# LauraFJulia/TFT_vs_Fund

Measured on AMD Instinct MI355X. Metric: triplet-hypotheses/sec (linearTFT+R,t) at N=200 corresp., higher is better.
Workload: dtype f64; 1 GPU; configs[1]: batch of 10000 synthetic triplets x 200 correspondences, sigma=1px, linearTFT + R_t_from_TFT (LinearTFTPoseEstimation without Reconst), one batch per GPU; batch_per_gpu=10000, correspondences=200, streams=2 (consecutive batches alternate between streams and may overlap), gather=none (1 GPU), failed_triplets=0, warmup_steps_run=2560

## Files before the change

tft_vs_fund_amd/csrc/gh_rows_kernel.h:

```cpp
#pragma once
#include "tft_rows_kernel.h"
#include "tft_rows_exact_kernel.h"
#include "gh_wg_kernel.h"

namespace tff {

template <bool PRE>
__global__ void __launch_bounds__(64, 2) k_gh_linear_rows(const GhWgArgs a) {
    TFF_DYNAMIC_LDS(double, smem);
    const int lane = lane_id();
    const int p = lane & 15, row = lane >> 4;
    RowLds* w = reinterpret_cast<RowLds*>(smem) + row;
    for (long blk = blockIdx.x; blk * ROW_TRIPLETS < a.B; blk += gridDim.x) {
        const int N = opaque_int(a.N);
        const long b_raw = blk * ROW_TRIPLETS + row;
        const bool valid = b_raw < a.B;
        const long b = valid ? b_raw : a.B - 1;
        RowSrc src;
        src.idx = nullptr; src.pts = a.corresp + b * 6 * (long)N; src.ns = 0; src.sampled = false;
        wave_sync();
        int status = ST_OK;
        if (N < 7) {
            status = ST_TOO_FEW;
        } else {
            if constexpr (PRE) {
                rows_load_pre(a.pre, b, w->mom, w->nrm);
            } else {
                double cen[6], nr[9];
                rows_centroids(src, N, cen);
                rows_distances_moments(src, N, cen, w->nrm, nr, w->mom);
            }
            wave_sync();
            const bool ok = rows_linear_tft_middle(w, nullptr, true);
            if (!ok) status = ST_RETRY;
            if (valid && ok) {
                double* r = a.rec + b * GH_REC_DOUBLES;
                r[p] = w->t[p];
                if (p < 11) r[16 + p] = w->t[16 + p];
                r[27 + p] = w->pa[p];
                if (p < 2) r[27 + 16 + p] = w->pa[16 + p];
                if (p < 6) r[45 + p] = w->epi[p];
                if (p < 9) r[51 + p] = w->nrm[p];
            }
        }
        if (p == 0 && valid) { a.status[b] = status; if (a.iter) a.iter[b] = 0; }
    }
}

__global__ void __launch_bounds__(64, 2) k_gh_finish_rows(const GhWgArgs a) {
    TFF_DYNAMIC_LDS(double, smem);
    const int lane = lane_id();
    const int p = lane & 15, row = lane >> 4;
    RowLds* w = reinterpret_cast<RowLds*>(smem) + row;
    RowRt* rt = reinterpret_cast<RowRt*>(w->ov);
    LinearTftArgs la{};
    la.corresp = a.corresp; la.calm = a.calm; la.calm_stride = a.calm_stride; la.B = a.B; la.N = a.N; la.flags = a.flags;
    la.Rt2 = a.Rt2; la.Rt3 = a.Rt3; la.T = a.T; la.reconst = a.reconst; la.iter = nullptr; la.status = a.status; la.dbg = nullptr;
    for (long blk = blockIdx.x; blk * ROW_TRIPLETS < a.B; blk += gridDim.x) {
        const int N = opaque_int(a.N);
        RowJob j;
        const long b_raw = blk * ROW_TRIPLETS + row;
        j.valid = b_raw < a.B;
        j.b = j.valid ? b_raw : a.B - 1;
        j.bad_index = false; j.dbg = nullptr;
        j.src.idx = nullptr; j.src.pts = a.corresp + j.b * 6 * (long)N; j.src.ns = 0; j.src.sampled = false;
        wave_sync();
        const int s0 = a.status[j.b];
        const bool dead = s0 > 0;
        if (dead) rows_store_nan(la, j, N);
        w->calm[p] = a.calm[j.b * a.calm_stride + p];
        if (p < 11) w->calm[16 + p] = a.calm[j.b * a.calm_stride + 16 + p];
        w->t[p] = dead ? ((p == 0) ? 1.0 : 0.0) : a.topt[j.b * 27 + p];
        if (p < 11) w->t[16 + p] = dead ? 0.0 : a.topt[j.b * 27 + 16 + p];
        if (p < 9) w->nrm[p] = dead ? ((p % 3 == 0) ? 1.0 : 0.0) : a.rec[j.b * GH_REC_DOUBLES + 51 + p];
        wave_sync();
        j.valid = j.valid && !dead;
        rows_transform_tft_inverse(w->t, rt->T1, rt->mats, [w](int v) { return normal_matrix(w->nrm, v); });
        bool ok = rows_rt_prepare<false>(w, rt, nullptr);
        int status = rows_pose_tail<false, false>(la, w, rt, j, N, ok);
        if (wave_any(status == ST_RETRY)) {
            RowJob jx = j;
            jx.valid = j.valid && status == ST_RETRY;
            wave_sync();
            rows_transform_tft_inverse(w->t, rt->T1, rt->mats, [w](int v) { return normal_matrix(w->nrm, v); });
            ok = rows_rt_prepare<true>(w, rt, nullptr);
            const int sx = rows_pose_tail<false, true>(la, w, rt, jx, N, ok);
            status = (status == ST_RETRY) ? sx : status;
        }
        if (s0 < 0) status = -s0;
        if (p == 0 && j.valid) a.status[j.b] = status;
    }
}

}
```

tft_vs_fund_amd/csrc/tft_rows_kernel.h:

```cpp
#pragma once
#include "tft_kernel.h"
#include "tft_moments_kernel.h"
#include <rows_target.h>
#include <regs_target.h>

namespace tff {

constexpr int ROW_TRIPLETS = 4;
constexpr int ROWL = 16;

struct RowRt {
    double T1[28];
    double T2[28];
    double nullv[18];
    double mats[28];
    double Ein[18];
    double cand[2][21];
    alignas(16) double P[4][12];
    alignas(16) double candRt[4][12];
    alignas(16) double Rt[2][12];
    alignas(16) double Pfin[3][12];
};
constexpr int ROW_OV_DOUBLES = 380;
static_assert(sizeof(RowRt) <= ROW_OV_DOUBLES * sizeof(double), "overlay");
struct alignas(16) RowLds {
    alignas(16) double mom[96];
    double nrm[9];
    double calm[27];
    double t[27];
    double epi[6];
    double Q[18];
    double tp[15];
    double pa[18];
    alignas(16) double ov[ROW_OV_DOUBLES];
};
static_assert(sizeof(RowLds) == (96 + 9 + 27 + 27 + 6 + 18 + 15 + 18 + ROW_OV_DOUBLES) * sizeof(double), "alignment adds no padding");
static_assert(sizeof(RowRt) == 318 * sizeof(double) && alignof(RowRt) == 16, "alignment adds no padding");
constexpr int ROW_LDS_DOUBLES = (int)(sizeof(RowLds) / sizeof(double));
static_assert(ROW_LDS_DOUBLES % 2 == 0, "16-byte row stride");
inline size_t rows_lds_bytes() { return (size_t)ROW_TRIPLETS * sizeof(RowLds); }
inline unsigned rows_grid(long B) { const long g = (B + ROW_TRIPLETS - 1) / ROW_TRIPLETS; return (unsigned)(g > 0 ? g : 1); }

__device__ __forceinline__ int rows_p() { return lane_id() & 15; }

struct RowSrc { const double* pts; const int* idx; int ns; bool sampled; };
__device__ __forceinline__ Pt6 rows_load(const RowSrc& s, const int i) {
    if (s.sampled) {
        int k = s.idx[i];
        k = (k >= 0 && k < s.ns) ? k : 0;
        return load_pt(s.pts, k);
    }
    return load_pt(s.pts, i);
}

__device__ __forceinline__ void rows_stamp(double* dbg, const int slot) {
    if (dbg) {
        const long long t = shader_clock();
        if (rows_p() == 0) dbg[80 + slot] = (double)t;
    }
}


__device__ __forceinline__ void rows_centroids(const RowSrc& s, const int N, double (&c)[6]) {
    const int p = rows_p();
    double sm[6] = {0, 0, 0, 0, 0, 0};
    int i0 = 0;
#pragma unroll 1
    for (; i0 + 4 * ROWL <= N; i0 += 4 * ROWL) {
        Pt6 q[4];
#pragma unroll
        for (int u = 0; u < 4; ++u) q[u] = rows_load(s, i0 + ROWL * u + p);
#pragma unroll
        for (int u = 0; u < 4; ++u)
#pragma unroll
            for (int k = 0; k < 6; ++k) sm[k] += q[u].v[k];
    }
    if (i0 < N) {
        Pt6 q[4];
#pragma unroll
        for (int u = 0; u < 4; ++u) { const int i = i0 + ROWL * u + p; q[u] = rows_load(s, (i < N) ? i : 0); }
#pragma unroll
        for (int u = 0; u < 4; ++u) {
            if (i0 + ROWL * u + p < N) {
#pragma unroll
                for (int k = 0; k < 6; ++k) sm[k] += q[u].v[k];
            }
        }
    }
#pragma unroll
    for (int k = 0; k < 6; ++k) c[k] = row_sum16(sm[k]) / (double)N;
}

__device__ __forceinline__ void rows_distances_moments(const RowSrc& s, const int N, const double (&c)[6], double* nrm, double (&nr)[9], double* mom) {
    const int p = rows_p();
    const int slot = p >> 1;
    const bool odd = (p & 1) != 0;
    double acc[48];
#pragma unroll
    for (int k = 0; k < 48; ++k) acc[k] = zero_f64();
    double dA = 0.0, dB = 0.0;
    auto body = [&](const Pt6& q, double& r2_out) {
        const double x1 = q.v[0] - c[0], y1 = q.v[1] - c[1];
        const double x2 = q.v[2] - c[2], y2 = q.v[3] - c[3];
        const double x3 = q.v[4] - c[4], y3 = q.v[5] - c[5];
        const double r1 = x1 * x1 + y1 * y1, r2 = x2 * x2 + y2 * y2, r3 = x3 * x3 + y3 * y3;
        dA += sqrt_nonneg_uniform(odd ? r3 : r1);
        r2_out = r2;
        const double q2[4] = {1.0, x2, y2, r2};
        const double q3[4] = {1.0, x3, y3, r3};
        const double pa = odd ? y1 * y1 : x1 * x1, pb = odd ? y1 : x1 * y1, pc = odd ? 1.0 : x1;
#pragma unroll
        for (int b = 0; b < 4; ++b)
#pragma unroll
            for (int cc = 0; cc < 4; ++cc) {
                const double wv = q3[b] * q2[cc];
                acc[4 * b + cc] += pa * wv;
                acc[16 + 4 * b + cc] += pb * wv;
                acc[32 + 4 * b + cc] += pc * wv;
            }
    };
    constexpr int STEP = ROWL / 2;
    Pt6 pe = rows_load(s, (slot < N) ? slot : 0);
    Pt6 po = rows_load(s, (slot + STEP < N) ? slot + STEP : 0);
#pragma unroll 1
    for (int i = slot; i < N; i += 2 * STEP) {
        const Pt6 q = pe;
        if (i + 2 * STEP < N) pe = rows_load(s, i + 2 * STEP);
        double r2a, r2b = 0.0;
        body(q, r2a);
        if (i + STEP < N) {
            const Pt6 r = po;
            if (i + 3 * STEP < N) po = rows_load(s, i + 3 * STEP);
            body(r, r2b);
        }
        dB += sqrt_nonneg_uniform(odd ? r2b : r2a);
    }
    const double d1 = row_sum16(odd ? 0.0 : dA), d3 = row_sum16(odd ? dA : 0.0), d2 = row_sum16(dB);
    const double r2c = sqrt(2.0);
    const double dd[3] = {d1, d2, d3};
#pragma unroll
    for (int v = 0; v < 3; ++v) {
        const double norm0 = dd[v] / (double)N;
        nr[3 * v + 0] = r2c / norm0;
        nr[3 * v + 1] = -r2c * c[2 * v] / norm0;
        nr[3 * v + 2] = -r2c * c[2 * v + 1] / norm0;
    }
    if (p == 0) {
#pragma unroll
        for (int k = 0; k < 9; ++k) nrm[k] = nr[k];
    }
    const bool up8 = (p & 8) != 0, up4 = (p & 4) != 0, up2 = (p & 2) != 0;
#pragma unroll
    for (int i = 0; i < 24; ++i) acc[i] = halve_sum<8>(acc[i], acc[i + 24], up8);
#pragma unroll
    for (int i = 0; i < 12; ++i) acc[i] = halve_sum<4>(acc[i], acc[i + 12], up4);
#pragma unroll
    for (int i = 0; i < 6; ++i) acc[i] = halve_sum<2>(acc[i], acc[i + 6], up2);
    const int base = 6 * ((p >> 1) & 1) + 12 * ((p >> 2) & 1) + 24 * ((p >> 3) & 1);
    const double s1 = nr[0], s2 = nr[3], s3 = nr[6];
#pragma unroll
    for (int i = 0; i < 6; ++i) {
        const int e = 48 * (p & 1) + base + i;
        const int h = e >> 4, i3 = (e >> 2) & 3, i2 = e & 3;
        const double f1 = (h == 5) ? 1.0 : ((h == 2 || h == 4) ? s1 : s1 * s1);
        const double f3 = (i3 == 0) ? 1.0 : ((i3 == 3) ? s3 * s3 : s3);
        const double f2 = (i2 == 0) ? 1.0 : ((i2 == 3) ? s2 * s2 : s2);
        mom[e] = acc[i] * (f1 * f3 * f2);
    }
}

template <int n>
__device__ __forceinline__ void rows_min_eigvec(double (&g0)[RowEigDims<n>::N0], double (&g1)[RowEigDims<n>::N1], const double d0, const double d1,
                                                double* Lp, const int maxit, int* iters, double* resid2, const bool has_start,
                                                const double start0, const double start1, double* gram_risk, double& x0, double& x1,
                                                const double gram_risk_limit2 = 1e14) {
    constexpr int N0 = RowEigDims<n>::N0;
    constexpr bool HI = RowEigDims<n>::HI;
    constexpr int Z = n * (n - 1) / 2;
    const int p = rows_p();
    const bool valid0 = p < n, valid1 = HI && 16 + p < n;
    const double tr = row_sum16((valid0 ? d0 : 0.0) + (valid1 ? d1 : 0.0));
    const double delta = 1e-14 * tr;
    const double pfloor = 1e-3 * delta + 1e-300;
    double myinv0 = 0.0, myinv1 = 0.0;
    RowChol<n, 0>::run(g0, g1, myinv0, myinv1, delta, pfloor, p);
#pragma unroll
    for (int c = 0; c < N0; ++c) g0[c] = (c < p && valid0) ? g0[c] * myinv0 : 0.0;
    if constexpr (HI) {
#pragma unroll
        for (int c = 0; c < n; ++c) g1[c] = ((c < 16 || c < 16 + p) && valid1) ? g1[c] * myinv1 : 0.0;
    }
    wave_sync();
    {
        const int t0 = (p * (p - 1)) / 2, t1 = ((16 + p) * (15 + p)) / 2;
#pragma unroll
        for (int c = 0; c < N0; ++c) Lp[(c < p && valid0) ? t0 + c : Z] = g0[c];
        if constexpr (HI) {
#pragma unroll
            for (int c = 0; c < n - 1; ++c) Lp[((c < 16 || c < 16 + p) && valid1) ? t1 + c : Z] = g1[c];
        }
    }
    wave_sync();
    x0 = valid0 ? rsqrt((double)n) : 0.0;
    x1 = valid1 ? rsqrt((double)n) : 0.0;
    if (has_start) {
        const double s0 = valid0 ? start0 : 0.0, s1 = valid1 ? start1 : 0.0;
        const double nn0 = row_sum16(s0 * s0 + s1 * s1);
        if (nn0 > 1e-300 && nn0 < 1e300) { const double r0 = rsqrt(nn0); x0 = s0 * r0; x1 = s1 * r0; }
    }
    double c0[n], c1[n];
#pragma unroll
    for (int j = 0; j < n; ++j) {
        c0[j] = Lp[(valid0 && p < j) ? (j * (j - 1)) / 2 + p : Z];
        c1[j] = (HI && j > 16) ? Lp[(valid1 && 16 + p < j) ? (j * (j - 1)) / 2 + 16 + p : Z] : 0.0;
    }
    double rprev2 = 1.0, res = 1.0, rk_r2 = 0.0, rk_rp = 1.0, rk_nn = 0.0;
    int it = 0;
    bool done = false;
#pragma unroll 1
    while (true) {
        double y0 = x0 * myinv0, y1 = x1 * myinv1;
        if constexpr (HI) {
            const double* rows = Lp + opaque_int(0);
            const int t0 = (p * (p - 1)) / 2;
#pragma unroll
            for (int c = 0; c < N0; ++c) g0[c] = rows[(c < p) ? t0 + c : Z];
        }
        RowForward<n, 0>::run(y0, y1, g0, g1);
        RowBackward<n, n - 1>::run(y0, y1, c0, c1);
        y0 *= myinv0; y1 *= myinv1;
        const double nn = row_sum16(y0 * y0 + y1 * y1);
        const double dot = row_sum16(y0 * x0 + y1 * x1);
        const double rn = rsqrt(nn);
        const double sc = (dot < 0.0) ? -rn : rn;
        const double yn0 = y0 * sc, yn1 = y1 * sc;
        const double dd0 = yn0 - x0, dd1 = yn1 - x1;
        const double r2 = row_sum16(dd0 * dd0 + dd1 * dd1);
        if (!done) {
            x0 = yn0; x1 = yn1;
            ++it;
            if (r2 <= 1e-26) { res = 0.0; done = true; }
            else if (it >= 2 && r2 < 0.25 * rprev2 && r2 * r2 < 1e-26 * rprev2) { res = 0.0; done = true; }
            else if (!(r2 == r2) || it >= maxit) { res = (r2 == r2) ? r2 : 1.0; done = true; }
            if (it >= 2 && r2 > 1e-30) { rk_r2 = r2; rk_rp = rprev2; rk_nn = nn; }
            rprev2 = r2;
        }
        if (!wave_any(!done)) break;
    }
    *iters = it;
    *resid2 = res;
    if (gram_risk) {
        const double num = 4.0 * rk_nn * rk_r2 * rk_rp;
        const double d = rk_rp - rk_r2;
        const double den = (rk_r2 < rk_rp) ? d * d : 0.0;
        *gram_risk = (tr * tr * num < gram_risk_limit2 * den) ? 0.0 : 1.0;
    }
}

template <class MatFn>
__device__ __forceinline__ void rows_transform_tft_inverse(const double* to, double* tn, double* mats, MatFn matrix_of) {
    const int p = rows_p();
    if (p < 3) {
        Mat3 M = matrix_of(p);
        if (p > 0) M = mat3_inv(M);
#pragma unroll
        for (int r = 0; r < 3; ++r)
#pragma unroll
            for (int c = 0; c < 3; ++c) mats[9 * p + 3 * r + c] = M.m[r][c];
    }
    wave_sync();
    double val[2];
#pragma unroll
    for (int h = 0; h < 2; ++h) {
        const int e = 16 * h + p;
        const bool have = e < 27;
        const int ee = have ? e : 0;
        const int i = ee / 9, k = (ee % 9) / 3, j = ee % 3;
        const double m0 = mats[i], m1 = mats[3 + i], m2 = mats[6 + i];
        double v = 0.0;
#pragma unroll
        for (int c = 0; c < 3; ++c)
#pragma unroll
            for (int d = 0; d < 3; ++d) {
                const double mix = m0 * to[c + 3 * d] + m1 * to[c + 3 * d + 9] + m2 * to[c + 3 * d + 18];
                v += mats[9 + 3 * j + c] * mix * mats[18 + 3 * k + d];
            }
        val[h] = have ? v : 0.0;
    }
    const double nn = row_sum16(val[0] * val[0] + val[1] * val[1]);
    const double rs = rsqrt(nn);
    wave_sync();
    tn[p] = val[0] * rs;
    if (p < 11) tn[16 + p] = val[1] * rs;
    wave_sync();
}

__device__ __forceinline__ bool rows_linear_tft_middle(RowLds* w, double* dbg, const bool want_P = false) {
    const int p = opaque_lane_int(rows_p());
    bool ok = true;
    int it1 = 0, it2 = 0;
    {
        const bool hi = p < 11;
        double ga[27], gb[27], g0[16], da, db, r2, risk, x0, x1;
        gram_row27(w->mom, p, ga, da);
        gram_row27(w->mom, hi ? 16 + p : 0, gb, db);
#pragma unroll
        for (int c = 0; c < 16; ++c) g0[c] = ga[c];
        rows_stamp(dbg, 3);
        rows_min_eigvec<27>(g0, gb, da, hi ? db : 0.0, w->ov, EIG_MAXIT, &it1, &r2, false, 0.0, 0.0, &risk, x0, x1);
        ok = ok && eig_converged(r2) && risk == 0.0;
        wave_sync();
        w->t[p] = x0;
        if (hi) w->t[16 + p] = x1;
        wave_sync();
    }
    if (dbg) { dbg[p] = w->t[p]; if (p < 11) dbg[16 + p] = w->t[16 + p]; }
    rows_stamp(dbg, 4);
    const bool eok = epipoles_from_tensor<16, false>(w->t, w->ov, w->epi, false);
    ok = !row_any(!eok) && ok;
    rows_stamp(dbg, 5);
    if (dbg && p < 6) dbg[27 + p] = w->epi[p];
    if (p < 2) frame_of(w->epi + 3 * p, w->Q + 9 * p);
    wave_sync();
    double* Gp = w->ov;
    constexpr GpIndexTable gp_index = make_gp_index_table();
    const unsigned long long gw0 = gp_index.w[rows_p()][0], gw1 = gp_index.w[rows_p()][1];
    int trip = 0;
#pragma unroll 1
    for (int e = p; e < 120; e += ROWL, ++trip) {
        const unsigned gw = (unsigned)(((trip < 4) ? gw0 : gw1) >> (16 * (trip & 3)));
        double a2[3], a3[3], b2[3], b3[3], c2[4], c3[4];
        up_factors_jk(w->Q, (int)(gw & 3u), (int)((gw >> 2) & 3u), a2, a3);
        up_factors_jk(w->Q, (int)((gw >> 4) & 3u), (int)((gw >> 6) & 3u), b2, b3);
        cvec(a2, b2, c2);
        cvec(a3, b3, c3);
        Gp[e] = bilinear44(w->mom + 16 * (int)((gw >> 8) & 7u), c3, c2);
    }
    wave_sync();
    rows_stamp(dbg, 6);
    {
        double g[15], none[1] = {0.0}, diag = 0.0, x0, x1, r2, risk;
        const bool have = p < 15;
        const int r = have ? p : 0;
#pragma unroll
        for (int c = 0; c < 15; ++c) g[c] = (c <= r && have) ? Gp[tri_index(r, c)] : 0.0;
        diag = Gp[tri_index(r, r)];
        double tp0 = 0.0;
        if (have) {
            const int i = r / 5, m = r % 5, jj = (m < 3) ? 0 : m - 2, kk = (m < 3) ? m : 0;
#pragma unroll
            for (int k = 0; k < 3; ++k)
#pragma unroll
                for (int j = 0; j < 3; ++j) tp0 += w->Q[3 * j + jj] * w->Q[9 + 3 * k + kk] * w->t[j + 3 * k + 9 * i];
        }
        wave_sync();
        rows_min_eigvec<15>(g, none, diag, 0.0, w->ov, EIG_MAXIT, &it2, &r2, true, tp0, 0.0, &risk, x0, x1);
        ok = ok && eig_converged(r2) && risk == 0.0;
        if (have) w->tp[p] = x0;
        wave_sync();
    }
    rows_stamp(dbg, 7);
    {
        double tv[2];
#pragma unroll
        for (int h = 0; h < 2; ++h) {
            const int e = (16 * h + p < 27) ? 16 * h + p : 0;
            const int i = e / 9, k = (e % 9) / 3, j = e % 3;
            double acc = 0.0;
#pragma unroll
            for (int m = 0; m < 5; ++m) {
                const int jj = (m < 3) ? 0 : m - 2, kk = (m < 3) ? m : 0;
                acc += w->Q[3 * j + jj] * w->Q[9 + 3 * k + kk] * w->tp[5 * i + m];
            }
            tv[h] = acc;
        }
        wave_sync();
        w->t[p] = tv[0];
        if (p < 11) w->t[16 + p] = tv[1];
        wave_sync();
    }
    if (dbg) {
        dbg[33 + p] = w->t[p];
        if (p < 11) dbg[33 + 16 + p] = w->t[16 + p];
        if (p == 0) { dbg[69] = (double)it1; dbg[70] = (double)it2; }
    }
    if (want_P) {
        if (p < 3) {
            const int i = p;
            const double* e21 = w->epi; const double* e31 = w->epi + 3;
            double ai[3], bi[3];
            for (int j = 0; j < 3; ++j) ai[j] = w->t[j + 9 * i] * e31[0] + w->t[j + 3 + 9 * i] * e31[1] + w->t[j + 6 + 9 * i] * e31[2];
            const double ae = ai[0] * e21[0] + ai[1] * e21[1] + ai[2] * e21[2];
            for (int k = 0; k < 3; ++k) {
                const double tte = w->t[3 * k + 9 * i] * e21[0] + w->t[1 + 3 * k + 9 * i] * e21[1] + w->t[2 + 3 * k + 9 * i] * e21[2];
                bi[k] = e31[k] * ae - tte;
            }
            const double be = bi[0] * e31[0] + bi[1] * e31[1] + bi[2] * e31[2];
            const double n21 = e21[0] * e21[0] + e21[1] * e21[1] + e21[2] * e21[2];
            const double n31 = e31[0] * e31[0] + e31[1] * e31[1] + e31[2] * e31[2];
            const double c = -(ae + be) / (n21 + n31);
            for (int j = 0; j < 3; ++j) { w->pa[3 * i + j] = ai[j] + c * e21[j]; w->pa[9 + 3 * i + j] = bi[j] + c * e31[j]; }
        }
        wave_sync();
    }
    return ok;
}

__device__ __forceinline__ void rows_recover_prepare(RowLds* w, RowRt* rt);
template <bool EXACT = false>
__device__ __forceinline__ bool rows_rt_prepare(RowLds* w, RowRt* rt, double* dbg) {
    const int p = rows_p();
    rows_transform_tft_inverse(rt->T1, rt->T2, rt->mats, [w](int v) { return load_K(w->calm, v); });
    const bool eok = epipoles_from_tensor<16, EXACT>(rt->T2, rt->nullv, w->epi, true);
    const bool ok = !row_any(!eok);
    if (p < 2) {
        const double* e21 = w->epi; const double* e31 = w->epi + 3;
        Mat3 M;
#pragma unroll
        for (int i = 0; i < 3; ++i)
#pragma unroll
            for (int r = 0; r < 3; ++r) {
                double acc = 0.0;
#pragma unroll
                for (int q = 0; q < 3; ++q) acc += (p == 0) ? rt->T2[r + 3 * q + 9 * i] * e31[q] : rt->T2[q + 3 * r + 9 * i] * e21[q];
                M.m[r][i] = acc;
            }
        const double* e = (p == 0) ? e21 : e31;
        const double sg = (p == 0) ? 1.0 : -1.0;
#pragma unroll
        for (int c = 0; c < 3; ++c) {
            rt->Ein[9 * p + 0 + c] = sg * (-e[2] * M.m[1][c] + e[1] * M.m[2][c]);
            rt->Ein[9 * p + 3 + c] = sg * (e[2] * M.m[0][c] - e[0] * M.m[2][c]);
            rt->Ein[9 * p + 6 + c] = sg * (-e[1] * M.m[0][c] + e[0] * M.m[1][c]);
        }
    }
    wave_sync();
    rows_stamp(dbg, 9);
    rows_recover_prepare(w, rt);
    return ok;
}

__device__ __forceinline__ void rows_recover_prepare(RowLds* w, RowRt* rt) {
    const int p = rows_p();
    if (p < 2) {
        Mat3 E, U, V;
#pragma unroll
        for (int r = 0; r < 3; ++r)
#pragma unroll
            for (int c = 0; c < 3; ++c) E.m[r][c] = rt->Ein[9 * p + 3 * r + c];
        double sv[3];
        svd3(E, U, V, sv);
        Mat3 UW, UWt, Vt = mat3_T(V);
#pragma unroll
        for (int r = 0; r < 3; ++r) {
            UW.m[r][0] = U.m[r][1];  UW.m[r][1] = -U.m[r][0]; UW.m[r][2] = U.m[r][2];
            UWt.m[r][0] = -U.m[r][1]; UWt.m[r][1] = U.m[r][0]; UWt.m[r][2] = U.m[r][2];
        }
        Mat3 R = mat3_mul(UW, Vt), Rp = mat3_mul(UWt, Vt);
        const double sR = sgn(mat3_det(R)), sRp = sgn(mat3_det(Rp));
        double* c = rt->cand[p];
#pragma unroll
        for (int r = 0; r < 3; ++r)
#pragma unroll
            for (int cc = 0; cc < 3; ++cc) { c[3 * r + cc] = R.m[r][cc] * sR; c[9 + 3 * r + cc] = Rp.m[r][cc] * sRp; }
        c[18] = U.m[0][2]; c[19] = U.m[1][2]; c[20] = U.m[2][2];
    }
    wave_sync();
    if (p < 4) {
        const int call = p >> 1, cd = p & 1;
        const Mat3 K = load_K(w->calm, call + 1);
        compose_camera(K, rt->cand[call] + 9 * cd, rt->cand[call] + 18, rt->P[p]);
#pragma unroll
        for (int r = 0; r < 3; ++r) {
#pragma unroll
            for (int c = 0; c < 3; ++c) rt->candRt[p][4 * r + c] = rt->cand[call][9 * cd + 3 * r + c];
            rt->candRt[p][4 * r + 3] = rt->cand[call][18 + r];
        }
    }
    if (p == 4) {
        const Mat3 K1 = load_K(w->calm, 0);
#pragma unroll
        for (int r = 0; r < 3; ++r) { rt->Pfin[0][4 * r] = K1.m[r][0]; rt->Pfin[0][4 * r + 1] = K1.m[r][1]; rt->Pfin[0][4 * r + 2] = K1.m[r][2]; rt->Pfin[0][4 * r + 3] = 0.0; }
    }
    wave_sync();
}

struct RowScale { double num, den; bool conv; bool main1[2]; };
template <bool SPEC = false>
__device__ __forceinline__ bool rows_votes(const RowSrc& s, const int N, const RowRt* rt, const bool all4, int (&sc)[2][2], int* sweeps_out = nullptr,
                                           bool* cert_out = nullptr, RowScale* scale = nullptr) {
    const int p = rows_p();
    double PA[12];
#pragma unroll
    for (int c = 0; c < 12; ++c) PA[c] = rt->Pfin[0][c];
    int scA[2] = {0, 0}, scB[2] = {0, 0};
    bool certA[2] = {true, true}, certB[2] = {true, true};
    int offA[2] = {0, 24}, offB[2] = {12, 36};
    bool main1[2] = {false, false};
    bool evalA = true, evalB[2] = {true, true};
    bool fullB[2] = {true, true};
    bool rowB[2] = {true, true};
    int sweeps = 0;
    double snum = 0.0, sden = 0.0;
    bool sconv = true;
#pragma unroll 1
    for (int sweep = 0; sweep < 2; ++sweep) {
        ++sweeps;
        const int start = (sweep == 0) ? 0 : ROWL;
        Pt6 pnext = rows_load(s, (start + p < N) ? start + p : 0);
#pragma unroll 1
        for (int i0 = start; i0 < N; i0 += ROWL) {
            const Pt6 q = pnext;
            const bool have = i0 + p < N;
            pnext = rows_load(s, (i0 + ROWL + p < N) ? i0 + ROWL + p : 0);
            const double x1 = q.v[0], y1 = q.v[1];
            double a0[3], a1[3], SA[6];
#pragma unroll
            for (int c = 0; c < 3; ++c) { a0[c] = y1 * PA[8 + c] - PA[4 + c]; a1[c] = PA[c] - x1 * PA[8 + c]; }
#pragma unroll
            for (int rr = 0; rr < 3; ++rr)
#pragma unroll
                for (int c = 0; c <= rr; ++c) SA[rr * (rr + 1) / 2 + c] = fma(a0[rr], a0[c], a1[rr] * a1[c]);
            const bool first = sweep == 0 && i0 == 0;
#pragma unroll
            for (int cc = 0; cc < 2; ++cc) {
                const int call = 1 - cc;
                const double x2 = (call == 0) ? q.v[2] : q.v[4], y2 = (call == 0) ? q.v[3] : q.v[5];
                VoteFactor fA, fB;
                if (evalA) {
                    VoteCam cam;
                    const int off = opaque_lane_int(offA[call]);
                    load_pairs16<12>(rt->P[0] + off, cam.PB);
                    load_pairs16<4>(rt->candRt[0] + off + 8, cam.R3);
                    int term = 0;
                    bool cert = true;
                    if (SPEC && call == 0 && !first) vote_one<true, false>(SA, cam, x2, y2, term, cert, &fA);
                    else if (SPEC && call == 0) vote_one<true>(SA, cam, x2, y2, term, cert, &fA);
                    else vote_one(SA, cam, x2, y2, term, cert);
                    scA[call] += have ? term : 0;
                    certA[call] = certA[call] && (cert || !have);
                }
                if (evalB[call]) {
                    VoteCam cam;
                    const int off = opaque_lane_int(offB[call]);
                    load_pairs16<12>(rt->P[0] + off, cam.PB);
                    load_pairs16<4>(rt->candRt[0] + off + 8, cam.R3);
                    int term = 0;
                    bool cert = true;
                    if (SPEC && call == 0 && first) vote_one<true>(SA, cam, x2, y2, term, cert, &fB);
                    else vote_one(SA, cam, x2, y2, term, cert);
                    scB[call] += have ? term : 0;
                    certB[call] = certB[call] && (cert || !have);
                }
                if (first) {
                    const bool v0 = row_any(have && certA[call] && scA[call] != 2), v1 = row_any(have && certA[call] && scA[call] != -2);
                    const bool b0 = row_any(have && certB[call] && scB[call] != 2), b1 = row_any(have && certB[call] && scB[call] != -2);
                    const bool mixA = v0 && v1, mixB = b0 && b1;
                    const bool single = !all4 && (mixA != mixB);
                    main1[call] = single && mixA;
                    if (main1[call]) {
                        const int ts = scA[call]; scA[call] = scB[call]; scB[call] = ts;
                        const bool tc = certA[call]; certA[call] = certB[call]; certB[call] = tc;
                        offA[call] = 12 + 24 * call; offB[call] = 24 * call;
                        if (SPEC && call == 0) fA = fB;
                    }
                    rowB[call] = !single;
                    evalB[call] = wave_any(!single);
                    fullB[call] = evalB[call];
                }
                if (SPEC && call == 0 && evalA) {
                    double X[4];
                    const bool conv = dlt_from_vote(fA, X);
                    sconv = sconv && (conv || !have);
                    if (!first) {
                        double pr[4];
                        load_pairs16<4>(rt->candRt[0] + opaque_lane_int(offA[0]) + 8, pr);
                        const double s4 = sgn(X[3]);
                        const double d1 = X[2] * s4, d2 = (pr[0] * X[0] + pr[1] * X[1] + pr[2] * X[2] + pr[3] * X[3]) * s4;
                        scA[0] += have ? sgn_i(d1) + sgn_i(d2) : 0;
                        certA[0] = certA[0] && (conv || !have);
                    }
                    const double iw = 1.0 / X[3];
                    const double X0 = X[0] * iw, X1 = X[1] * iw, X2 = X[2] * iw;
                    double ax[12];
                    load_pairs16<12>(rt->P[0] + opaque_lane_int(offA[1]), ax);
                    double X3[3], u3[3];
#pragma unroll
                    for (int r = 0; r < 3; ++r) { X3[r] = ax[4 * r] * X0 + ax[4 * r + 1] * X1 + ax[4 * r + 2] * X2; u3[r] = ax[4 * r + 3]; }
                    const double p3[3] = {q.v[4], q.v[5], 1.0};
                    double c1[3], c2[3];
                    cross3(p3, X3, c1);
                    cross3(p3, u3, c2);
                    snum += have ? c1[0] * c2[0] + c1[1] * c2[1] + c1[2] * c2[2] : 0.0;
                    sden += have ? c2[0] * c2[0] + c2[1] * c2[1] + c2[2] * c2[2] : 0.0;
                }
            }
        }
        if (sweep == 1) break;
        bool again = false;
#pragma unroll
        for (int call = 0; call < 2; ++call) {
            const int tA = (int)row_sum16((double)scA[call]);
            const bool mine = !rowB[call] && tA != 2 * N && tA != -2 * N;
            rowB[call] = rowB[call] || mine;
            const bool need = wave_any(!fullB[call] && tA != 2 * N && tA != -2 * N);
            evalB[call] = need;
            fullB[call] = fullB[call] || need;
            again = again || need;
        }
        evalA = false;
        if (!again) break;
    }
    bool ok = true;
#pragma unroll
    for (int call = 0; call < 2; ++call) {
        const int tA = (int)row_sum16((double)scA[call]);
        const int tBsum = (int)row_sum16((double)scB[call]);
        const int tB = (fullB[call] && rowB[call]) ? tBsum : 0;
        const bool badA = row_any(!certA[call]), badB = row_any(!certB[call]);
        ok = ok && !badA && (!(fullB[call] && rowB[call]) || !badB);
        if (cert_out) {
            cert_out[2 * call] = main1[call] ? !badB : !badA;
            cert_out[2 * call + 1] = main1[call] ? !badA : !badB;
        }
        sc[call][0] = main1[call] ? tB : tA;
        sc[call][1] = main1[call] ? tA : tB;
    }
    if constexpr (SPEC) {
        scale->num = row_sum16(snum);
        scale->den = row_sum16(sden);
        scale->conv = !row_any(!sconv);
        scale->main1[0] = main1[0];
        scale->main1[1] = main1[1];
    }
    if (sweeps_out) *sweeps_out = sweeps + (fullB[0] ? 16 : 0) + (fullB[1] ? 32 : 0);
    return ok;
}

template <int MODE, bool EXACT = false>
__device__ __forceinline__ bool rows_tri_pass(const RowSrc& s, const int N, const double* camA, const double* camB, const double* aux,
                                              double* out, double& num_out, double& den_out) {
    const int p = rows_p();
    double PAr[12], PBr[12], AXr[12];
    if (!EXACT) {
#pragma unroll
        for (int c = 0; c < 12; ++c) { PAr[c] = camA[c]; PBr[c] = camB[c]; AXr[c] = aux[c]; }
    }
    typedef const double (&cam_ref)[12];
    cam_ref PA = EXACT ? *reinterpret_cast<const double(*)[12]>(camA) : PAr;
    cam_ref PB = EXACT ? *reinterpret_cast<const double(*)[12]>(camB) : PBr;
    cam_ref AX = EXACT ? *reinterpret_cast<const double(*)[12]>(aux) : AXr;
    bool all_conv = true;
    double num = 0.0, den = 0.0;
    Pt6 pnext = rows_load(s, (p < N) ? p : 0);
#pragma unroll 1
    for (int i = p; i < N; i += ROWL) {
        const Pt6 q = pnext;
        if (i + ROWL < N) pnext = rows_load(s, i + ROWL);
        double X[4];
        const bool conv = dlt_point<EXACT, EXACT>(PA, PB, AX, camA, camB, aux, MODE == TRI_RECONST, q.v[0], q.v[1], q.v[2], q.v[3], q.v[4], q.v[5], X);
        all_conv = all_conv && conv;
        const double iw = 1.0 / X[3];
        const double X0 = X[0] * iw, X1 = X[1] * iw, X2 = X[2] * iw;
        if constexpr (MODE == TRI_SCALE) {
            double X3[3];
#pragma unroll
            for (int r = 0; r < 3; ++r) X3[r] = AX[4 * r] * X0 + AX[4 * r + 1] * X1 + AX[4 * r + 2] * X2;
            const double u3[3] = {AX[3], AX[7], AX[11]};
            const double p3[3] = {q.v[4], q.v[5], 1.0};
            double c1[3], c2[3];
            cross3(p3, X3, c1);
            cross3(p3, u3, c2);
            num += c1[0] * c2[0] + c1[1] * c2[1] + c1[2] * c2[2];
            den += c2[0] * c2[0] + c2[1] * c2[1] + c2[2] * c2[2];
        } else if (out) {
            out[3 * (long)i + 0] = X0;
            out[3 * (long)i + 1] = X1;
            out[3 * (long)i + 2] = X2;
        }
    }
    if constexpr (MODE == TRI_SCALE) {
        num_out = row_sum16(num);
        den_out = row_sum16(den);
    }
    return !row_any(!all_conv);
}

struct RowJob {
    long b;
    bool valid;
    bool bad_index;
    double* dbg;
    RowSrc src;
    long base = 0;
};
__device__ __forceinline__ RowJob rows_begin(const LinearTftArgs& a, RowLds* w, const long blk, const int N) {
    const int lane = lane_id(), p = lane & 15, row = lane >> 4;
    RowJob j;
    const long b_raw = blk * ROW_TRIPLETS + row;
    j.valid = b_raw < a.B;
    j.b = j.valid ? b_raw : a.B - 1;
    j.dbg = a.dbg ? a.dbg + j.b * DBG_STRIDE : nullptr;
    j.src.idx = a.sample_idx ? a.sample_idx + j.b * (long)N : nullptr;
    j.src.pts = a.sample_idx ? a.corresp : a.corresp + j.b * 6 * (long)N;
    j.src.ns = a.sample_ns;
    j.src.sampled = a.sample_idx != nullptr;
    wave_sync();
    j.bad_index = false;
    if (a.sample_idx) {
        bool bad = false;
        for (int i = p; i < N; i += ROWL) { const int k = j.src.idx[i]; bad = bad || !(k >= 0 && k < j.src.ns); }
        j.bad_index = row_any(bad);
    }
    w->calm[p] = a.calm[j.b * a.calm_stride + p];
    if (p < 11) w->calm[16 + p] = a.calm[j.b * a.calm_stride + 16 + p];
    return j;
}
__device__ __forceinline__ long rows_ragged_slot(const LinearTftArgs& a, const long blk) { return a.rrange[0] + blk * ROW_TRIPLETS; }
__device__ __forceinline__ int rows_ragged_n(const LinearTftArgs& a, const long blk) {
    const long b0 = a.rlist[rows_ragged_slot(a, blk)];
    return opaque_int(wave_uniform_i((int)(a.offsets[b0 + 1] - a.offsets[b0])));
}
__device__ __forceinline__ RowJob rows_begin_ragged(const LinearTftArgs& a, RowLds* w, const long blk) {
    const int lane = lane_id(), p = lane & 15, row = lane >> 4;
    const long slot = rows_ragged_slot(a, blk);
    const int e = a.rlist[slot + row];
    RowJob j;
    j.valid = e >= 0;
    j.b = j.valid ? (long)e : (long)a.rlist[slot];
    j.base = a.offsets[j.b];
    j.dbg = nullptr;
    j.src.idx = nullptr;
    j.src.pts = a.corresp + 6 * j.base;
    j.src.ns = 0;
    j.src.sampled = false;
    wave_sync();
    j.bad_index = false;
    w->calm[p] = a.calm[j.b * a.calm_stride + p];
    if (p < 11) w->calm[16 + p] = a.calm[j.b * a.calm_stride + 16 + p];
    return j;
}
template <bool KERNARG>
__device__ __forceinline__ auto rows_args_at(const LinearTftArgs& a) {
    if constexpr (KERNARG) return kernarg_again(a);
    else return &a;
}
template <bool RAGGED = false, bool KERNARG = false>
__device__ __forceinline__ void rows_store_nan(const LinearTftArgs& a, const RowJob& j, const int N) {
    const int p = rows_p();
    const double qnan = __longlong_as_double(0x7ff8000000000000LL);
    if (j.valid) {
        const auto* al = rows_args_at<KERNARG>(a);
        double* const oRt2 = al->Rt2; double* const oRt3 = al->Rt3; double* const oT = al->T; double* const orec = al->reconst;
        if (p < 12) { oRt2[j.b * 12 + p] = qnan; oRt3[j.b * 12 + p] = qnan; }
        oT[j.b * 27 + p] = qnan;
        if (p < 11) oT[j.b * 27 + 16 + p] = qnan;
        if (orec) for (int i = p; i < 3 * N; i += ROWL) orec[(RAGGED ? 3 * j.base : j.b * 3 * (long)N) + i] = qnan;
    }
}

__device__ __forceinline__ int rows_vote_exact(const RowSrc& s, const int N, const RowRt* rt, const int cand_off, const int view) {
    const int p = rows_p();
    typedef const double (&cam_ref)[12];
    cam_ref PA = *reinterpret_cast<const double(*)[12]>(rt->Pfin[0]);
    const double* camB = rt->P[0] + cand_off;
    cam_ref PB = *reinterpret_cast<const double(*)[12]>(camB);
    const double* pr = rt->candRt[0] + cand_off;
    double score = 0.0;
#pragma unroll 1
    for (int i = p; i < N; i += ROWL) {
        const Pt6 q = rows_load(s, i);
        double X[4];
        dlt_point<true, true>(PA, PB, PB, rt->Pfin[0], camB, camB, false, q.v[0], q.v[1], (view == 1) ? q.v[2] : q.v[4], (view == 1) ? q.v[3] : q.v[5], 0.0, 0.0, X);
        const double s4 = sgn(X[3]);
        const double d1 = X[2] * s4, d2 = (pr[8] * X[0] + pr[9] * X[1] + pr[10] * X[2] + pr[11] * X[3]) * s4;
        score += sgn(d1) + sgn(d2);
    }
    return (int)row_sum16(score);
}

__device__ __forceinline__ void rows_vote_exact_pair(const RowSrc& s, const int N, const RowRt* rt, const int k, const int view, int& exA, int& exB) {
    const int p = rows_p(), half = p >> 3, i = p & 7;
    const int cand_off = 12 * (k + half);
    typedef const double (&cam_ref)[12];
    cam_ref PA = *reinterpret_cast<const double(*)[12]>(rt->Pfin[0]);
    const double* camB = rt->P[0] + cand_off;
    cam_ref PB = *reinterpret_cast<const double(*)[12]>(camB);
    const double* pr = rt->candRt[0] + cand_off;
    double score = 0.0;
    if (i < N) {
        const Pt6 q = rows_load(s, i);
        double X[4];
        dlt_point<true, true>(PA, PB, PB, rt->Pfin[0], camB, camB, false, q.v[0], q.v[1], (view == 1) ? q.v[2] : q.v[4], (view == 1) ? q.v[3] : q.v[5], 0.0, 0.0, X);
        const double s4 = sgn(X[3]);
        const double d1 = X[2] * s4, d2 = (pr[8] * X[0] + pr[9] * X[1] + pr[10] * X[2] + pr[11] * X[3]) * s4;
        score = sgn(d1) + sgn(d2);
    }
    exA = (int)row_sum16(half ? 0.0 : score);
    exB = (int)row_sum16(half ? score : 0.0);
}

template <bool T_FROM_CAMERAS, bool EXACT = false, bool RAGGED = false, bool KERNARG = false>
__device__ __forceinline__ int rows_pose_tail(const LinearTftArgs& a, RowLds* w, RowRt* rt, const RowJob& j, const int N, bool ok) {
    const int p = rows_p();
    double* dbg = j.dbg;
    const long b = j.b;
    int status = ST_OK;
    RowScale spec;
    spec.num = 0.0; spec.den = 1.0; spec.conv = true; spec.main1[0] = spec.main1[1] = false;
    bool spec_valid = !EXACT;
    double spec_sign = 1.0;
    {
        int sc[2][2];
        int sweeps = 0;
        if constexpr (EXACT) {
            bool cert4[4];
            rows_votes(j.src, N, rt, true, sc, &sweeps, cert4);
            rows_stamp(dbg, 3);
            if (N <= 8) {
#pragma unroll 1
                for (int call = 0; call < 2; ++call) {
                    const bool needA = !(call ? cert4[2] : cert4[0]), needB = !(call ? cert4[3] : cert4[1]);
                    if (!wave_any(needA || needB)) continue;
                    int exA, exB;
                    rows_vote_exact_pair(j.src, N, rt, 2 * call, call + 1, exA, exB);
                    if (needA) { if (call) sc[1][0] = exA; else sc[0][0] = exA; }
                    if (needB) { if (call) sc[1][1] = exB; else sc[0][1] = exB; }
                }
            } else {
#pragma unroll 1
                for (int k = 0; k < 4; ++k) {
                    const bool need = !((k == 0) ? cert4[0] : (k == 1) ? cert4[1] : (k == 2) ? cert4[2] : cert4[3]);
                    if (!wave_any(need)) continue;
                    const int ex = rows_vote_exact(j.src, N, rt, 12 * k, (k < 2) ? 1 : 2);
                    if (need) { if (k == 0) sc[0][0] = ex; else if (k == 1) sc[0][1] = ex; else if (k == 2) sc[1][0] = ex; else sc[1][1] = ex; }
                }
            }
        } else {
            ok = rows_votes<true>(j.src, N, rt, dbg != nullptr && !(a.flags & FLAG_DBG_ADAPTIVE), sc, &sweeps, nullptr, &spec) && ok;
        }
        if (dbg && p == 0) dbg[94] = (double)sweeps;
#pragma unroll
        for (int call = 0; call < 2; ++call) {
            const int sR = sc[call][0], sRp = sc[call][1];
            const int score[4] = {sR, -sR, -sRp, sRp};
            int seen = 0, pick = -1;
#pragma unroll
            for (int k = 0; k < 4; ++k) if (score[k] >= seen) { pick = k; seen = score[k]; }
            if (pick < 0) status = ST_NO_POSE;
            if (dbg && p < 4) dbg[60 + 4 * call + p] = (double)((p == 0) ? score[0] : (p == 1) ? score[1] : (p == 2) ? score[2] : score[3]);
            if (p < 12) {
                const int r = p >> 2, c = p & 3;
                const double* R = rt->cand[call] + ((pick >= 2) ? 9 : 0);
                const double tsign = (pick == 1 || pick == 2) ? -1.0 : 1.0;
                rt->Rt[call][p] = (c < 3) ? R[3 * r + c] : tsign * rt->cand[call][18 + r];
            }
            spec_valid = spec_valid && pick >= 0 && ((pick >= 2) == spec.main1[call]);
            spec_sign = (pick == 1 || pick == 2) ? -spec_sign : spec_sign;
        }
        wave_sync();
    }
    rows_stamp(dbg, 11);
    {
        if (p < 2) compose_camera_from_pose(load_K(w->calm, p + 1), rt->Rt[p], rt->Pfin[p + 1]);
        wave_sync();
        double num = spec_sign * spec.num, den = spec.den;
        bool conv = spec.conv;
        if (dbg && p == 0) dbg[95] = spec_valid ? 1.0 : 0.0;
        if (wave_any(!spec_valid)) {
            double n2, d2;
            const bool c2 = rows_tri_pass<TRI_SCALE, EXACT>(j.src, N, rt->Pfin[0], rt->Pfin[1], rt->Pfin[2], nullptr, n2, d2);
            if (!spec_valid) { num = n2; den = d2; conv = c2; }
        }
        ok = ok && conv;
        const double lam = -num / den;
        if (dbg && p == 0) dbg[68] = lam;
        if (p < 3) rt->Rt[1][4 * p + 3] *= lam;
        wave_sync();
    }
    rows_stamp(dbg, 12);
    double* const oreconst = rows_args_at<KERNARG>(a)->reconst;
    if (oreconst || T_FROM_CAMERAS) {
        if (p == 0) compose_camera_from_pose(load_K(w->calm, 2), rt->Rt[1], rt->Pfin[2]);
        wave_sync();
    }
    if constexpr (T_FROM_CAMERAS) {
        double val[2];
#pragma unroll
        for (int h = 0; h < 2; ++h) {
            const int e = (16 * h + p < 27) ? 16 * h + p : 0;
            const int i = e / 9, k = (e % 9) / 3, jj = e % 3;
            const int r0 = (i == 0) ? 1 : 0, r1 = (i == 2) ? 1 : 2;
            double m[4][4];
#pragma unroll
            for (int c = 0; c < 4; ++c) {
                m[0][c] = rt->Pfin[0][4 * r0 + c];
                m[1][c] = rt->Pfin[0][4 * r1 + c];
                m[2][c] = rt->Pfin[1][4 * jj + c];
                m[3][c] = rt->Pfin[2][4 * k + c];
            }
            val[h] = (16 * h + p < 27) ? ((i == 1) ? -1.0 : 1.0) * det4(m) : 0.0;
        }
        const double rs = rsqrt(row_sum16(val[0] * val[0] + val[1] * val[1]));
        rt->T1[p] = val[0] * rs;
        if (p < 11) rt->T1[16 + p] = val[1] * rs;
        wave_sync();
    }
    double vRt[2], vT[2];
    bool bad = false;
#pragma unroll
    for (int h = 0; h < 2; ++h) {
        const int e24 = 16 * h + p;
        vRt[h] = 0.0; vT[h] = 0.0;
        if (e24 < 24) {
            const int which = e24 / 12, e = e24 % 12, c = e / 3, r = e % 3;
            vRt[h] = rt->Rt[which][4 * r + c];
        }
        if (e24 < 27) vT[h] = rt->T1[e24];
        bad = bad || !(fabs(vRt[h]) <= 1.79e308) || !(fabs(vT[h]) <= 1.79e308);
    }
    const bool nonfinite = row_any(bad);
    if (oreconst) {
        double n0, d0;
        double* rec = (j.valid && !j.bad_index && !nonfinite) ? oreconst + (RAGGED ? 3 * j.base : b * 3 * (long)N) : nullptr;
        const bool conv = rows_tri_pass<TRI_RECONST, EXACT>(j.src, N, rt->Pfin[0], rt->Pfin[1], rt->Pfin[2], rec, n0, d0);
        ok = ok && conv;
    }
    if (j.bad_index) status = ST_TOO_FEW;
    else if (!ok) status = ST_RETRY;
    else if (nonfinite && status == ST_OK) status = ST_NONFINITE;
    if (j.bad_index || (ok && nonfinite)) {
        rows_store_nan<RAGGED, KERNARG>(a, j, N);
    } else {
        const bool store = j.valid && ok;
        auto stores = [&](const auto* al) {
            double* const oRt2 = al->Rt2; double* const oRt3 = al->Rt3; double* const oT = al->T;
#pragma unroll
            for (int h = 0; h < 2; ++h) {
                const int e24 = 16 * h + p;
                if (e24 < 24 && store) ((e24 >= 12) ? oRt3 : oRt2)[b * 12 + e24 % 12] = vRt[h];
                if (e24 < 27 && store) oT[b * 27 + e24] = vT[h];
            }
        };
        stores(rows_args_at<KERNARG>(a));
    }
    rows_stamp(dbg, 13);
    return status;
}

template <bool PRE, bool RAGGED = false>
__global__ void __launch_bounds__(64, 2) k_linear_tft_pose_rows(const LinearTftArgs a) {
    TFF_DYNAMIC_LDS(double, smem);
    if (a.retry_zero && blockIdx.x == 0 && threadIdx.x == 0) *a.retry_zero = 0;
    const int p = lane_id() & 15, row = lane_id() >> 4;
    RowLds* w = reinterpret_cast<RowLds*>(smem) + row;
    RowRt* rt = reinterpret_cast<RowRt*>(w->ov);
    for (long blk = blockIdx.x; RAGGED ? rows_ragged_slot(a, blk) < a.rrange[1] : blk * ROW_TRIPLETS < a.B; blk += gridDim.x) {
        const int N = RAGGED ? rows_ragged_n(a, blk) : opaque_int(a.N);
        const RowJob j = RAGGED ? rows_begin_ragged(a, w, blk) : rows_begin(a, w, blk, N);
        double* dbg = j.dbg;
        rows_stamp(dbg, 0);
        int status;
        if (N < 7) {
            status = ST_TOO_FEW;
            rows_store_nan<RAGGED, true>(a, j, N);
        } else {
            if constexpr (PRE) {
                rows_load_pre(a.pre, j.b, w->mom, w->nrm);
                rows_stamp(dbg, 1);
                wave_sync();
                if (dbg && p < 9) dbg[71 + p] = w->nrm[p];
            } else {
                double cen[6], nr[9];
                rows_centroids(j.src, N, cen);
                rows_stamp(dbg, 1);
                rows_distances_moments(j.src, N, cen, w->nrm, nr, w->mom);
                if (dbg && p < 9) dbg[71 + p] = w->nrm[p];
            }
            wave_sync();
            rows_stamp(dbg, 2);
            bool ok = rows_linear_tft_middle(w, dbg);
            rows_stamp(dbg, 8);
            rows_transform_tft_inverse(w->t, rt->T1, rt->mats, [w](int v) { return normal_matrix(w->nrm, v); });
            ok = rows_rt_prepare(w, rt, dbg) && ok;
            rows_stamp(dbg, 10);
            status = rows_pose_tail<false, false, RAGGED, true>(a, w, rt, j, N, ok);
        }
        if (p == 0 && j.valid) {
            const auto* al = kernarg_again(a);
            int* const oiter = al->iter; int* const ostatus = al->status; int* const olist = al->retry_list;
            if (oiter) oiter[j.b] = 0;
            ostatus[j.b] = status;
            if (status == ST_RETRY && olist) olist[atomicAdd(al->retry_count, 1)] = (int)j.b;
        }
    }
}

}
```

Baseline: 104.3 million triplet-hypotheses/s.

## Reduce moment accumulators through LDS transpose and double-buffer point loads

Replaces the shuffle-based halving reduction of the 48 per-lane moment accumulators with a chunked LDS transpose through the overlay scratch: each lane writes its partials, then reads and sums eight peers' values for two output entries. The point-load loop is restructured into a ping-pong of two prefetch buffer pairs, with empty asm barriers that force the previous loads to land before the next ones are issued. The squared-radius computations now use an fma. This cuts cross-lane shuffle traffic in exchange for LDS round trips and extra wave syncs, and it adds register pressure from the extra buffers.

After: 106.1 million triplet-hypotheses/s, median of 6. +1.8%, better.

```diff
diff --git a/tft_vs_fund_amd/csrc/gh_rows_kernel.h b/tft_vs_fund_amd/csrc/gh_rows_kernel.h
--- a/tft_vs_fund_amd/csrc/gh_rows_kernel.h
+++ b/tft_vs_fund_amd/csrc/gh_rows_kernel.h
@@ -28,7 +28,7 @@
             } else {
                 double cen[6], nr[9];
                 rows_centroids(src, N, cen);
-                rows_distances_moments(src, N, cen, w->nrm, nr, w->mom);
+                rows_distances_moments(src, N, cen, w->nrm, nr, w->mom, w->ov);
             }
             wave_sync();
             const bool ok = rows_linear_tft_middle(w, nullptr, true);
diff --git a/tft_vs_fund_amd/csrc/moments_target.h b/tft_vs_fund_amd/csrc/moments_target.h
--- /dev/null
+++ b/tft_vs_fund_amd/csrc/moments_target.h
@@ -0,0 +1,14 @@
+#pragma once
+#include <hip/hip_runtime.h>
+
+namespace tff {
+
+__device__ __forceinline__ double sum_sq_yx(double x, double y) { return fma(y, y, x * x); }
+
+template <int N>
+__device__ __forceinline__ void loads_landed(const double (&v)[N]) {
+#pragma unroll
+    for (int k = 0; k < N; ++k) asm volatile("" ::"v"(v[k]));
+}
+
+}
diff --git a/tft_vs_fund_amd/csrc/tft_rows_kernel.h b/tft_vs_fund_amd/csrc/tft_rows_kernel.h
--- a/tft_vs_fund_amd/csrc/tft_rows_kernel.h
+++ b/tft_vs_fund_amd/csrc/tft_rows_kernel.h
@@ -3,6 +3,7 @@
 #include "tft_moments_kernel.h"
 #include <rows_target.h>
 #include <regs_target.h>
+#include <moments_target.h>
 
 namespace tff {
 
@@ -91,7 +92,7 @@
     for (int k = 0; k < 6; ++k) c[k] = row_sum16(sm[k]) / (double)N;
 }
 
-__device__ __forceinline__ void rows_distances_moments(const RowSrc& s, const int N, const double (&c)[6], double* nrm, double (&nr)[9], double* mom) {
+__device__ __forceinline__ void rows_distances_moments(const RowSrc& s, const int N, const double (&c)[6], double* nrm, double (&nr)[9], double* mom, double* ov) {
     const int p = rows_p();
     const int slot = p >> 1;
     const bool odd = (p & 1) != 0;
@@ -103,7 +104,7 @@
         const double x1 = q.v[0] - c[0], y1 = q.v[1] - c[1];
         const double x2 = q.v[2] - c[2], y2 = q.v[3] - c[3];
         const double x3 = q.v[4] - c[4], y3 = q.v[5] - c[5];
-        const double r1 = x1 * x1 + y1 * y1, r2 = x2 * x2 + y2 * y2, r3 = x3 * x3 + y3 * y3;
+        const double r1 = sum_sq_yx(x1, y1), r2 = sum_sq_yx(x2, y2), r3 = sum_sq_yx(x3, y3);
         dA += sqrt_nonneg_uniform(odd ? r3 : r1);
         r2_out = r2;
         const double q2[4] = {1.0, x2, y2, r2};
@@ -120,20 +121,24 @@
             }
     };
     constexpr int STEP = ROWL / 2;
-    Pt6 pe = rows_load(s, (slot < N) ? slot : 0);
-    Pt6 po = rows_load(s, (slot + STEP < N) ? slot + STEP : 0);
+    auto trip = [&](const Pt6& ce, const Pt6& co, Pt6& ne, Pt6& no, const int i) {
+        loads_landed(ce.v);
+        loads_landed(co.v);
+        if (i + 2 * STEP < N) ne = rows_load(s, i + 2 * STEP);
+        if (i + 3 * STEP < N) no = rows_load(s, i + 3 * STEP);
+        double r2a, r2b = 0.0;
+        body(ce, r2a);
+        if (i + STEP < N) body(co, r2b);
+        dB += sqrt_nonneg_uniform(odd ? r2b : r2a);
+    };
+    Pt6 ae = rows_load(s, (slot < N) ? slot : 0);
+    Pt6 ao = rows_load(s, (slot + STEP < N) ? slot + STEP : 0);
+    Pt6 be = ae, bo = ao;
 #pragma unroll 1
-    for (int i = slot; i < N; i += 2 * STEP) {
-        const Pt6 q = pe;
-        if (i + 2 * STEP < N) pe = rows_load(s, i + 2 * STEP);
-        double r2a, r2b = 0.0;
-        body(q, r2a);
-        if (i + STEP < N) {
-            const Pt6 r = po;
-            if (i + 3 * STEP < N) po = rows_load(s, i + 3 * STEP);
-            body(r, r2b);
-        }
-        dB += sqrt_nonneg_uniform(odd ? r2b : r2a);
+    for (int i0 = 0; i0 < N; i0 += 4 * STEP) {
+        if (i0 + slot < N) trip(ae, ao, be, bo, i0 + slot);
+        if (i0 + 2 * STEP >= N) break;
+        if (i0 + 2 * STEP + slot < N) trip(be, bo, ae, ao, i0 + 2 * STEP + slot);
     }
     const double d1 = row_sum16(odd ? 0.0 : dA), d3 = row_sum16(odd ? dA : 0.0), d2 = row_sum16(dB);
     const double r2c = sqrt(2.0);
@@ -149,23 +154,33 @@
 #pragma unroll
         for (int k = 0; k < 9; ++k) nrm[k] = nr[k];
     }
-    const bool up8 = (p & 8) != 0, up4 = (p & 4) != 0, up2 = (p & 2) != 0;
-#pragma unroll
-    for (int i = 0; i < 24; ++i) acc[i] = halve_sum<8>(acc[i], acc[i + 24], up8);
-#pragma unroll
-    for (int i = 0; i < 12; ++i) acc[i] = halve_sum<4>(acc[i], acc[i + 12], up4);
-#pragma unroll
-    for (int i = 0; i < 6; ++i) acc[i] = halve_sum<2>(acc[i], acc[i + 6], up2);
-    const int base = 6 * ((p >> 1) & 1) + 12 * ((p >> 2) & 1) + 24 * ((p >> 3) & 1);
+    constexpr int CH = 16, LSTRIDE = CH + 2;
+    static_assert(48 % CH == 0 && ROWL * LSTRIDE <= ROW_OV_DOUBLES && (LSTRIDE * sizeof(double)) % 16 == 0, "chunks fit the overlay, pairs stay aligned");
+    const int par = p & 1;
+    Pair16* const mine = reinterpret_cast<Pair16*>(ov + LSTRIDE * p);
+    const double* const theirs = ov + LSTRIDE * par + 2 * (p >> 1);
     const double s1 = nr[0], s2 = nr[3], s3 = nr[6];
-#pragma unroll
-    for (int i = 0; i < 6; ++i) {
-        const int e = 48 * (p & 1) + base + i;
-        const int h = e >> 4, i3 = (e >> 2) & 3, i2 = e & 3;
-        const double f1 = (h == 5) ? 1.0 : ((h == 2 || h == 4) ? s1 : s1 * s1);
-        const double f3 = (i3 == 0) ? 1.0 : ((i3 == 3) ? s3 * s3 : s3);
-        const double f2 = (i2 == 0) ? 1.0 : ((i2 == 3) ? s2 * s2 : s2);
-        mom[e] = acc[i] * (f1 * f3 * f2);
+    const int i3 = (p >> 2) & 3;
+    const bool i2hi = ((p >> 1) & 1) != 0;
+    const double f3 = (i3 == 0) ? 1.0 : ((i3 == 3) ? s3 * s3 : s3);
+    const double f2[2] = {i2hi ? s2 : 1.0, i2hi ? s2 * s2 : s2};
+    const double f1c[3] = {s1 * s1, par ? s1 : s1 * s1, par ? 1.0 : s1};
+#pragma unroll
+    for (int c = 0; c < 48 / CH; ++c) {
+        if (c > 0) wave_sync();
+#pragma unroll
+        for (int k = 0; k < CH; k += 2) { Pair16 v; v[0] = acc[CH * c + k]; v[1] = acc[CH * c + k + 1]; mine[k / 2] = v; }
+        wave_sync();
+        double v[8][2];
+#pragma unroll
+        for (int m = 0; m < 8; ++m) load_pairs16<2>(theirs + 2 * LSTRIDE * m, v[m]);
+        Pair16 out;
+#pragma unroll
+        for (int t = 0; t < 2; ++t) {
+            const double sum = ((v[0][t] + v[4][t]) + (v[2][t] + v[6][t])) + ((v[1][t] + v[5][t]) + (v[3][t] + v[7][t]));
+            out[t] = sum * (f1c[c] * f3 * f2[t]);
+        }
+        *reinterpret_cast<Pair16*>(mom + 48 * par + CH * c + 2 * (p >> 1)) = out;
     }
 }
 
@@ -974,7 +989,7 @@
                 double cen[6], nr[9];
                 rows_centroids(j.src, N, cen);
                 rows_stamp(dbg, 1);
-                rows_distances_moments(j.src, N, cen, w->nrm, nr, w->mom);
+                rows_distances_moments(j.src, N, cen, w->nrm, nr, w->mom, w->ov);
                 if (dbg && p < 9) dbg[71 + p] = w->nrm[p];
             }
             wave_sync();
```
